# sdmiller/cpu_tsdf

Hardware: AMD Instinct MI355X
Metric: integrateCloud throughput, Scene A turntable depth frames, 640x480 -> voxel grid (higher is better)
Workload: dtype f32

## Files before the change

### cpu_tsdf_amd/csrc/tsdf_common.h

```cpp
#pragma once

#include <hip/hip_runtime.h>
#include <stdint.h>
#include <cmath>
#include <string>
#include <vector>

#include "tsdf_hip.h"

struct tsdf_hip_pipeline;
struct tsdf_hip_multi;
struct tsdf_occ_state;
struct tsdf_meshpost_state;
struct tsdf_flatten_state;
struct tsdf_esdf_state;

struct tsdf_hip_volume {
  tsdf_hip_multi *multi = nullptr;
  tsdf_params p;
  int device = 0;
  int nx = 0, ny = 0, nz = 0;
  int z_begin = 0, z_end = 0;
  int z_first = 0;
  int nz_alloc = 0;
  int64_t pitch = 0;
  int levels[3] = {0, 0, 0};
  float *d = nullptr, *w = nullptr;
  uint32_t *rgb = nullptr;
  uint8_t *k8 = nullptr;
  float *cn[4] = {nullptr, nullptr, nullptr, nullptr};
  float *lab_lut = nullptr;
  float4 *lab_img = nullptr;
  float *vm = nullptr;
  int32_t *vn = nullptr;
  int expf_fused_r = 0;
  float alloc_probe_ms[8] = {-1.f, -1.f, -1.f, -1.f, -1.f, -1.f, -1.f, -1.f};
  int alloc_tried = 0, alloc_chosen = 0;
  int packed = 0;
  unsigned kmax = 0;
  int weight_by_depth = 0, weight_by_variance = 0;
  float *ctr[3] = {nullptr, nullptr, nullptr};
  std::vector<float> h_ctr[3];
  float *frame_depth = nullptr;
  uint32_t *frame_bgra = nullptr;
  uint2 *frame_pairs[2] = {nullptr, nullptr};
  char *bounce = nullptr;
  hipEvent_t bounce_ev[2] = {nullptr, nullptr};
  bool bounce_busy[2] = {false, false};
  unsigned bounce_turn = 0;
  double *cam64 = nullptr;
  tsdf_hip_pipeline *pipe = nullptr;
  int frame_staged = 0;
  uint8_t *band = nullptr;
  int band_fx = 0, band_fy = 0;
  bool band_exact = false;
  int rest_state = 0;
  uint32_t rest_bits = 0;
  unsigned long long last_implied = 0, last_read_bytes = 0;
  bool last_implied_on = false;
  uint8_t *live = nullptr;
  size_t live_cap = 0;
  uint32_t *row_iv = nullptr;
  size_t row_iv_cap = 0;
  bool ctr_increasing[3] = {false, false, false};
  unsigned long long *counter = nullptr;
  unsigned long long last_observed = 0, last_changed_bytes = 0;
  bool ref_cull = false;
  float cull_planes[24] = {0};
// ... 209 lines not shown
int tsdf_shift_band(tsdf_hip_volume *v, int sx, int sy, int sz);
int tsdf_shift_mark(tsdf_hip_volume *v, int which);
void tsdf_shift_clamp(const tsdf_hip_volume *v, const int32_t shift[3], int s[3]);
void tsdf_shift_count(int nx, int ny, int nz, const int s[3], uint64_t *kept, uint64_t *reset);

struct TsdfTuning {
  int rows_per_block;
  int blocks_per_cu;
  int fast_projection;
  int mc_flush_at;
  int mc_skip;
  int cull;
  int vol_chunk;
  int plain_kernel;
  int alloc_tries;
  int allin;
  int refcull_plain;
  int live_log2tx;
  int zfast;
  int fuse2;
  int implied_d;
  int pipe;
  int lab_chunk;
  int frame_pairs;
};
const TsdfTuning &tsdf_tuning();
int tsdf_vol_chunk();

struct PlaneView {
  const float *d, *w;
  const uint32_t *rgb;
  const uint8_t *k8;
  float wmax;
  unsigned kmax;
  int packed;
};

static inline PlaneView tsdf_plane_view(const tsdf_hip_volume *v) {
  return PlaneView{v->d, v->w, v->rgb, v->k8, v->p.max_weight, v->kmax, v->packed};
}

static __device__ __forceinline__ float tsdf_decode_w(unsigned k, float wmax) {
  const float kf = (float)k;
  return kf > wmax ? wmax : kf;
}

// ... 28 lines not shown
```

### cpu_tsdf_amd/csrc/tsdf_core.hip

```cpp
#include <math.h>

#include <string>
#include <stdlib.h>
#include <stdio.h>

#include <algorithm>
#include <thread>
#include <string.h>

#include "tsdf_common.h"
#ifdef TSDF_HIP_TEST_HOOKS
#include "tsdf_hip_test.h"
#endif

static thread_local std::string g_last_error;

void tsdf_set_error(const std::string &msg) { g_last_error = msg; }

int tsdf_hip_fail(hipError_t e, const char *what, const char *file, int line) {
  char buf[512];
  snprintf(buf, sizeof buf, "%s:%d: %s -> %s", file, line, what, hipGetErrorString(e));
  g_last_error = buf;
  (void)hipGetLastError();
  return e == hipErrorOutOfMemory ? TSDF_HIP_E_NOMEM : TSDF_HIP_E_HIP;
}

extern "C" const char *tsdf_hip_last_error(void) { return g_last_error.c_str(); }

extern "C" const char *tsdf_hip_error_string(int code) {
  switch (code) {
    case TSDF_HIP_OK: return "ok";
    case TSDF_HIP_E_INVALID: return "invalid argument";
    case TSDF_HIP_E_NOMEM: return "out of device memory";
    case TSDF_HIP_E_HIP: return "HIP runtime error";
    case TSDF_HIP_E_NODEVICE: return "no HIP device";
    case TSDF_HIP_E_UNSUPPORTED: return "unsupported";
    case TSDF_HIP_E_IO: return "file error";
    case TSDF_HIP_ALIGN_NO_POINTS: return "alignment: no point passed the gate";
    case TSDF_HIP_ALIGN_RANK_DEFICIENT: return "alignment: the cloud does not constrain all six freedoms";
  }
  return "unknown";
}

static int env_int(const char *name, int dflt) {
  const char *e = getenv(name);
  return (e && *e) ? atoi(e) : dflt;
}

static TsdfTuning &tuning_storage() {
  static TsdfTuning t = {std::max(1, env_int("TSDF_HIP_ROWS_PER_BLOCK", 64)),
                         std::max(1, env_int("TSDF_HIP_BLOCKS_PER_CU", 8)),
                         env_int("TSDF_HIP_FAST_PROJECTION", -1), env_int("TSDF_HIP_MC_FLUSH_AT", 512), env_int("TSDF_HIP_MC_SKIP", 1),
                         env_int("TSDF_HIP_CULL", 1), std::max(1, env_int("TSDF_HIP_VOL_CHUNK", 256)),
                         env_int("TSDF_HIP_PLAIN_KERNEL", 0), env_int("TSDF_HIP_ALLOC_TRIES", 3), env_int("TSDF_HIP_ALLIN", 1),
                         env_int("TSDF_HIP_REFCULL_PLAIN", 0), env_int("TSDF_HIP_LIVE_LOG2TX", 5), env_int("TSDF_HIP_ZFAST", 1), env_int("TSDF_HIP_FUSE2", 1), env_int("TSDF_HIP_IMPLIED_D", 1),
                         env_int("TSDF_HIP_PIPE", 1), std::max(1, env_int("TSDF_HIP_LAB_CHUNK", 16 << 20)), env_int("TSDF_HIP_FRAME_PAIRS", 1)};
  return t;
}

const TsdfTuning &tsdf_tuning() { return tuning_storage(); }

int tsdf_vol_chunk() {
  const int live = env_int("TSDF_HIP_VOL_CHUNK", 0);
  return live > 0 ? live : tsdf_tuning().vol_chunk;
}

#ifdef TSDF_HIP_TEST_HOOKS
extern "C" int tsdf_hip_set_tuning(const char *name, int value) {
  if (!name) return TSDF_HIP_E_INVALID;
  TsdfTuning &t = tuning_storage();
  const std::string n(name);
  if (n == "rows_per_block")
    t.rows_per_block = std::max(1, value);
  else if (n == "blocks_per_cu")
    t.blocks_per_cu = std::max(1, value);
  else if (n == "fast_projection")
    t.fast_projection = value;
  else if (n == "mc_flush_at")
    t.mc_flush_at = value;
// ... 5 lines not shown
    t.vol_chunk = std::max(1, value);
  else if (n == "plain_kernel")
    t.plain_kernel = value;
  else if (n == "alloc_tries")
    t.alloc_tries = std::max(1, value);
  else if (n == "allin")
    t.allin = value;
  else if (n == "refcull_plain")
    t.refcull_plain = value;
  else if (n == "fuse2")
    t.fuse2 = value;
  else if (n == "implied_d")
    t.implied_d = value;
  else if (n == "pipe")
    t.pipe = value;
  else if (n == "live_log2tx")
    t.live_log2tx = value;
  else if (n == "zfast")
    t.zfast = value;
  else if (n == "lab_chunk")
    t.lab_chunk = std::max(1, value);
  else if (n == "frame_pairs")
    t.frame_pairs = value;
  else
    return TSDF_HIP_E_INVALID;
  return TSDF_HIP_OK;
}
#endif

extern "C" int tsdf_hip_abi_version(void) { return TSDF_HIP_ABI_VERSION; }

extern "C" int tsdf_hip_host_alloc(size_t bytes, void **out) {
  if (!out || !bytes) return TSDF_HIP_E_INVALID;
  *out = nullptr;
  TSDF_HIP_TRY(hipHostMalloc(out, bytes, hipHostMallocPortable));
  return TSDF_HIP_OK;
}

extern "C" int tsdf_hip_host_free(void *p) {
  if (!p) return TSDF_HIP_OK;
  TSDF_HIP_TRY(hipHostFree(p));
  return TSDF_HIP_OK;
}

extern "C" int tsdf_hip_device_count(void) {
  int n = 0;
// ... 238 lines not shown
  if (!v) return;
  tsdf_occupied_release(v);
  tsdf_meshpost_release(v);
  tsdf_flatten_release(v);
  tsdf_esdf_release(v);
  if (v->multi) tsdf_multi_free(v);
  TsdfDeviceScope scope(v->device);
  tsdf_pipeline_destroy(v);
  if (v->d) (void)hipFree(v->d);
  if (v->w) (void)hipFree(v->w);
  if (v->rgb) (void)hipFree(v->rgb);
  if (v->k8) (void)hipFree(v->k8);
  for (int c = 0; c < 4; ++c)
    if (v->cn[c]) (void)hipFree(v->cn[c]);
  if (v->vm) (void)hipFree(v->vm);
  if (v->vn) (void)hipFree(v->vn);
  if (v->lab_lut) (void)hipFree(v->lab_lut);
  if (v->lab_img) (void)hipFree(v->lab_img);
  for (int a = 0; a < 3; ++a)
    if (v->ctr[a]) (void)hipFree(v->ctr[a]);
  if (v->frame_depth) (void)hipFree(v->frame_depth);
  for (int i = 0; i < 2; ++i)
    if (v->frame_pairs[i]) (void)hipFree(v->frame_pairs[i]);
  if (v->bounce) (void)hipHostFree(v->bounce);
  for (int i = 0; i < 2; ++i)
    if (v->bounce_ev[i]) (void)hipEventDestroy(v->bounce_ev[i]);
  if (v->cam64) (void)hipFree(v->cam64);
  if (v->live) (void)hipFree(v->live);
  if (v->row_iv) (void)hipFree(v->row_iv);
  if (v->band) (void)hipFree(v->band);
  if (v->counter) (void)hipFree(v->counter);
  if (v->mc_verts) (void)hipFree(v->mc_verts);
  if (v->mc_rgb) (void)hipFree(v->mc_rgb);
  if (v->mc_cell) (void)hipFree(v->mc_cell);
  if (v->mc_keys) (void)hipFree(v->mc_keys);
  if (v->mc_vals) (void)hipFree(v->mc_vals);
  if (v->mc_need) (void)hipFree(v->mc_need);
  for (int i = 0; i < 4; ++i)
    if (v->mc_ev[i]) (void)hipEventDestroy(v->mc_ev[i]);
  for (int i = 0; i < 2; ++i)
    if (v->align_ev[i]) (void)hipEventDestroy(v->align_ev[i]);
  for (int i = 0; i < 2; ++i)
    if (v->shift_ev[i]) (void)hipEventDestroy(v->shift_ev[i]);
  for (int i = 0; i < 3; ++i)
    if (v->merge_ev[i]) (void)hipEventDestroy(v->merge_ev[i]);
  if (v->merge_count) (void)hipFree(v->merge_count);
// ... 220 lines not shown
    for (int c = 0; c < (lab ? 3 : 4); ++c) TRY_OR_BAIL(hipMalloc(&v->cn[c], n * sizeof(float)));
  if (lab) {
    float lut[256];
    tsdf_lab_curve(lut);
    TRY_OR_BAIL(hipMalloc(&v->lab_lut, sizeof lut));
    TRY_OR_BAIL(hipMemcpy(v->lab_lut, lut, sizeof lut, hipMemcpyHostToDevice));
    TRY_OR_BAIL(hipMalloc(&v->lab_img, (size_t)p->image_width * p->image_height * sizeof(float4)));
  }
  for (int a = 0; a < 3; ++a) {
    tsdf_build_centers(p->res[a], tsdf_node_size(*p, a), v->h_ctr[a], &v->levels[a]);
    v->ctr_increasing[a] = true;
    for (size_t i = 1; i < v->h_ctr[a].size(); ++i) v->ctr_increasing[a] &= v->h_ctr[a][i - 1] < v->h_ctr[a][i];
    std::vector<float> padded(v->h_ctr[a]);
    padded.resize((size_t)p->res[a] + 4, NAN);
    TRY_OR_BAIL(hipMalloc(&v->ctr[a], padded.size() * sizeof(float)));
    TRY_OR_BAIL(hipMemcpy(v->ctr[a], padded.data(), padded.size() * sizeof(float), hipMemcpyHostToDevice));
  }
  const size_t npx = (size_t)p->image_width * p->image_height;
  TRY_OR_BAIL(hipMalloc(&v->frame_depth, 2 * npx * sizeof(float)));
  v->frame_bgra = reinterpret_cast<uint32_t *>(v->frame_depth + npx);
  if (p->integrate_color)
    for (int i = 0; i < 2; ++i) TRY_OR_BAIL(hipMalloc(&v->frame_pairs[i], 8 * npx));
  {
    const double cam[4] = {p->fx, p->fy, p->cx, p->cy};
    TRY_OR_BAIL(hipMalloc(&v->cam64, sizeof cam));
    TRY_OR_BAIL(hipMemcpy(v->cam64, cam, sizeof cam, hipMemcpyHostToDevice));
  }
  v->band_fx = (v->nx + 63) / 64;
  v->band_fy = (v->ny + 3) / 4;
  TRY_OR_BAIL(hipMalloc(&v->band, (size_t)v->band_fx * v->band_fy * v->nz_alloc));
  TRY_OR_BAIL(hipMalloc(&v->counter, 4096 * sizeof(unsigned long long)));
  TRY_OR_BAIL(hipMemset(v->counter, 0, 4096 * sizeof(unsigned long long)));
#undef TRY_OR_BAIL
  rc = tsdf_hip_reset(v);
  if (rc != TSDF_HIP_OK) return bail(rc);
  *out = v;
  return TSDF_HIP_OK;
}

extern "C" int tsdf_hip_reset(tsdf_handle h) {
  if (!h) return TSDF_HIP_E_INVALID;
  tsdf_normals_invalidate(h);
  if (h->multi) return tsdf_multi_reset(h);
  TSDF_ENTER(h);
  const int64_t n = h->pitch * h->ny * h->nz_alloc;
  const float minus_one = -1.f;
// ... 490 lines not shown
```

### cpu_tsdf_amd/csrc/tsdf_integrate.hip

```cpp
#include <limits.h>
#include <string.h>
#include <math.h>

#include <algorithm>
#include <cmath>
#include <type_traits>

#include "tsdf_common.h"
#include "tsdf_div.h"
#include "tsdf_buffer.h"
#ifdef TSDF_HIP_TEST_HOOKS
#include "tsdf_hip_test.h"
#endif

#ifndef TSDF_WPE_MAX
#define TSDF_WPE_MAX 8
#endif
#ifndef TSDF_WPE_PACKED
#define TSDF_WPE_PACKED 7
#endif
#ifndef TSDF_WPE_PACKED_COLOR
#define TSDF_WPE_PACKED_COLOR 8
#endif
#ifndef TSDF_WPE_GENERAL
#define TSDF_WPE_GENERAL 7
#endif
#ifndef TSDF_WPE_PIPE
#define TSDF_WPE_PIPE 8
#endif
#ifndef TSDF_WPE_PIPEC
#define TSDF_WPE_PIPEC 5
#endif
#ifndef TSDF_WPE_K2
// ... 350 lines not shown
  TSDF_CNT2_READ = 2560,
  TSDF_CNT2_SLOTS = 3072
};
static __device__ __forceinline__ unsigned tsdf_block_number(const BlockCoords &bc) { return bc.bx + bc.by * bc.gdx + bc.bz * bc.gdx * bc.gdy; }
static __device__ __forceinline__ void tsdf_count_out(const BlockCoords &bc, unsigned *s, unsigned long long *n_obs,
                                                      unsigned tid, unsigned cnt, unsigned chg, unsigned imp, unsigned rdb) {
  if (tid == 0) s[0] = s[1] = s[2] = s[3] = 0;
  __syncthreads();
  if (cnt) atomicAdd(&s[0], cnt);
  if (chg) atomicAdd(&s[1], chg);
  if (imp) atomicAdd(&s[2], imp);
  if (rdb) atomicAdd(&s[3], rdb);
  __syncthreads();
  if (tid == 0 && (s[0] || s[3])) {
    const unsigned b = tsdf_block_number(bc) & (TSDF_CNT_STRIPE - 1u);
    if (s[0]) atomicAdd(n_obs + TSDF_CNT_OBSERVED + b, (unsigned long long)s[0]);
    if (s[1]) atomicAdd(n_obs + TSDF_CNT_CHANGED + b, (unsigned long long)s[1]);
    if (s[2]) atomicAdd(n_obs + TSDF_CNT_IMPLIED + b, (unsigned long long)s[2]);
    if (s[3]) atomicAdd(n_obs + TSDF_CNT_READ + b, (unsigned long long)s[3]);
  }
}
#define TSDF_WPE_OF(ORDER, COLOR, FASTPROJ, COUNT, PACKED, ALLIN) \
  ((ALLIN) && !(COUNT) && (PACKED) && (COLOR) && (FASTPROJ) ? TSDF_WPE_PACKED_COLOR : (ALLIN) && !(COUNT) && ((PACKED) || !(COLOR)) ? TSDF_WPE_PACKED : TSDF_WPE_GENERAL)
template <int ORDER, bool COLOR, bool FASTPROJ, bool COUNT, bool PACKED, bool ALLIN = false, bool LIVE = false, bool PAIRS = false>
static __global__ void __launch_bounds__(256) __attribute__((amdgpu_waves_per_eu(TSDF_WPE_OF(ORDER, COLOR, FASTPROJ, COUNT, PACKED, ALLIN) < TSDF_WPE_MAX ? TSDF_WPE_OF(ORDER, COLOR, FASTPROJ, COUNT, PACKED, ALLIN) : TSDF_WPE_MAX, TSDF_WPE_MAX)))
k_integrate(const IntegrateArgs a, float *__restrict__ D, float *__restrict__ Wt, uint32_t *__restrict__ RGB,
            uint8_t *__restrict__ K8, const float *__restrict__ depth, const double *__restrict__ cam,
            const float *__restrict__ ctrx, const float *__restrict__ ctry, const float *__restrict__ ctrz,
            unsigned long long *__restrict__ n_obs, const uint8_t *__restrict__ live, uint8_t *__restrict__ band,
            const uint32_t *__restrict__ row_iv) {
  static_assert(!(ALLIN && LIVE), "the ALLIN instance knows no row intervals");
  static_assert(!PAIRS || COLOR, "pixel records carry the colour: the colourless frame is the depth plane itself");
  const BlockCoords bc = tsdf_block_coords(a.zfast);
  bool strad = false;
  if (LIVE) {
    const unsigned flag = live[bc.bx + bc.gdx * (bc.by + bc.gdy * bc.bz)];
    if (flag == 0u) return;
    strad = flag == 2u;
  }
  const unsigned tid = threadIdx.x;
  __shared__ f2 s_rcp[256];
  __shared__ f4 s_yt[256];
  constexpr bool F2 = ALLIN && FASTPROJ;
  constexpr bool LEAN_K1 = PACKED && COLOR;
  __shared__ f4 s_cx[F2 ? 256 : 1];
  __shared__ uint32_t s_iv[LIVE ? 256 : 1];
  TSDF_BAND_DECL;
  if (PACKED) s_rcp[tid] = tsdf_rcp_entry(a, tid);
  {
    const int yy = (int)bc.by * a.rpb * a.TY + (int)tid;
    const float cy_ = ctry[yy < a.ny ? yy : a.ny - 1], cz_ = ctrz[a.z_global0 + (int)bc.bz];
    f4 t = {0.f, 0.f, 0.f, 0.f};
#pragma unroll
    for (int q = 0; q < 3; ++q) t[q] = tsdf_row_part<ORDER>(a.m, q, cy_, cz_);
    s_yt[tid] = t;
    if (LIVE && strad) s_iv[tid] = yy < a.ny ? row_iv[(int64_t)bc.bz * a.ny + yy] : 0u;
  }
  if (F2) tsdf_park_centres(a, bc, ctrx, s_cx, tid);
  __shared__ uint8_t s_bin[PACKED ? 1024 : 1];
  if (PACKED && a.implied_d) tsdf_flags_before(a, bc, band, s_bin, tid);
  __syncthreads();
  const uint64_t quiet = PACKED && a.implied_d ? tsdf_quiet_passes(a, s_bin, tid) : 0ull;
  const int tx = (int)(tid & (unsigned)(a.TX - 1));
  const int ty = (int)(tid >> a.log2TX);
  const int xq = (int)bc.bx * a.TX + tx;
  const int zl = (int)bc.bz;
  const Rcp32 rneg = rcp32_prepare(a.neg);
  unsigned cnt = 0, chg = 0, imp = 0, rdb = 0;
  const BlockRows br = tsdf_block_rows(a, bc);
  const rsrc_t rsD = make_rsrc(D + br.e0, br.span * 4u);
  const rsrc_t rsW = make_rsrc(PACKED ? D : Wt + br.e0, PACKED ? 0u : br.span * 4u);
  const rsrc_t rsC = make_rsrc(COLOR ? RGB + br.e0 : (uint32_t *)D, COLOR ? br.span * 4u : 0u);
  const rsrc_t rsK = make_rsrc(PACKED && !COLOR ? K8 + br.e0 : (uint8_t *)D, PACKED && !COLOR ? br.span : 0u);
  const unsigned npix = (unsigned)a.W * (unsigned)a.H;
  const rsrc_t rsF = make_rsrc(depth, PAIRS ? npix * 8u : COLOR ? a.bgra_off + npix * 4u : npix * 4u);
  const i4_rsrc rsFi = make_rsrc_2d(depth, PAIRS ? 8u : 4u, 0xffffffffu);
  if (xq < a.qpr) {
    const int x4 = xq * 4;
    const float cz = ctrz[a.z_global0 + zl];
    const float4 cx4 = *reinterpret_cast<const float4 *>(ctrx + x4);
    const float cxs[4] = {cx4.x, cx4.y, cx4.z, cx4.w};
    float px_[4][3], zt[3];
#pragma unroll
    for (int r = 0; r < 3; ++r) {
#pragma unroll
      for (int j = 0; j < 4; ++j) px_[j][r] = cxs[j] * a.m[4 * r];
      zt[r] = ORDER == TSDF_XFORM_PCL_SSE ? cz * a.m[4 * r + 2] + a.m[4 * r + 3] : a.m[4 * r + 2] * cz;
    }
    const unsigned voff = (unsigned)(ty * (int)a.pitch + x4) * 4u;
    const unsigned row_step = (unsigned)a.TY * (unsigned)a.pitch * 4u;
    bool pred_obs = true;
    for (int r = 0; r < a.rpb; ++r) {
      const int y = br.row0 + ty + r * a.TY;
      if (y >= a.ny) break;
      unsigned iv_lo = 0u, iv_len = 0u;
      if (LIVE && strad) {
        const uint32_t iv = s_iv[ty + r * a.TY];
        iv_lo = iv & 0xffffu, iv_len = iv >> 16;
        if (!((unsigned)(x4 + 3) - iv_lo < iv_len + 3u)) continue;
      }
      const unsigned soff = (unsigned)r * row_step;
      const f4 ytv = s_yt[ty + r * a.TY];
      const float yt[3] = {ytv.x, ytv.y, ytv.z};
      float px[4][3];
      if constexpr (!F2) {
        float cxr[4] = {cxs[0], cxs[1], cxs[2], cxs[3]};
#pragma unroll
        for (int j = 0; j < 4; ++j) asm volatile("" : "+v"(cxr[j]));
#pragma unroll
        for (int q = 0; q < 3; ++q)
#pragma unroll
          for (int j = 0; j < 4; ++j) px[j][q] = cxr[j] * a.m[4 * q];
      }
      auto transform = [&](int j, int q) -> float {
        if (ORDER == TSDF_XFORM_PCL_SSE) return px[j][q] + yt[q];
// ... 1553 lines not shown
static __global__ void __launch_bounds__(256)
k_frame_pairs(const uint32_t *__restrict__ depth, const uint32_t *__restrict__ bgra, uint2 *__restrict__ out, unsigned npix) {
  const unsigned i = (blockIdx.x * 256u + threadIdx.x) * 2u;
  if (i + 1u < npix) {
    const uint4 v = {depth[i], bgra[i], depth[i + 1u], bgra[i + 1u]};
    *reinterpret_cast<uint4 *>(out + i) = v;
  } else if (i < npix) {
    out[i] = make_uint2(depth[i], bgra[i]);
  }
}

static int launch_frame_pairs(tsdf_handle h, const float *d_depth, const uint32_t *d_bgra, uint2 *out) {
  const unsigned npix = (unsigned)h->p.image_width * (unsigned)h->p.image_height;
  if (!out || !d_depth || !d_bgra) {
    tsdf_set_error("colour launch without its pixel-record buffer or frame");
    return TSDF_HIP_E_INVALID;
  }
  hipLaunchKernelGGL(k_frame_pairs, dim3((npix + 511u) / 512u), dim3(256), 0, h->stream, reinterpret_cast<const uint32_t *>(d_depth),
                     d_bgra, out, npix);
  TSDF_HIP_TRY(hipGetLastError());
  return TSDF_HIP_OK;
}

static bool frame_pairs_apply(tsdf_handle h) { return tsdf_tuning().frame_pairs && h->p.integrate_color; }

static int zfast_for(const tsdf_params &p, unsigned gx) {
  const size_t frame_bytes = (size_t)p.image_width * p.image_height * (p.integrate_color ? 8 : 4);
  return tsdf_tuning().zfast < 0 ? (frame_bytes > (3u << 20) && gx <= 65535u) : (tsdf_tuning().zfast != 0 && gx <= 65535u);
}

static uint8_t *band_flags_for(tsdf_handle h, const IntegrateArgs &a) {
  uint8_t *band = h->band_exact && ((a.rpb * a.TY) & 3) == 0 && (a.y_abs0 & 3) == 0 ? h->band : nullptr;
  if (!band) h->band_exact = false;
  return band;
}

static bool pipelined_rows_apply(tsdf_handle h, const IntegrateArgs &a, bool color, bool fastproj, bool allin, bool live) {
  return (tsdf_tuning().pipe & (color ? 2 : 1)) && fastproj && allin && !live && h->packed && a.hinge_fixed && a.neg_in_window &&
         a.ny % a.TY == 0;
}

static int launch_plain_family(tsdf_handle h, const IntegrateArgs &a, unsigned gz, int plain_mode, const float *d_depth,
                               const uint32_t *d_bgra, const float T[12], bool count) {
  const tsdf_params &p = h->p;
  if (plain_mode && ((h->packed && plain_mode != 3) || h->cn[0])) {
    tsdf_set_error("weight_by_depth needs the F32W layout and TSDF_COLOR_RGB");
// ... 162 lines not shown
  if (const int e = grow_live_scratch(h, nb, nrows)) return e;
  const dim3 row_grid((unsigned)((nrows + 255) / 256)), block(256);
  if (ra.nx <= TSDF_ROWS_LDS_NX)
    hipLaunchKernelGGL(k_rows<true>, row_grid, block, 0, h->stream, ra, pl.ctrx, pl.ctry, h->ctr[2], h->row_iv);
  else
    hipLaunchKernelGGL(k_rows<false>, row_grid, block, 0, h->stream, ra, pl.ctrx, pl.ctry, h->ctr[2], h->row_iv);
  hipLaunchKernelGGL(k_cull, dim3((unsigned)((nb + 255) / 256)), block, 0, h->stream, c, pl.ctrx, pl.ctry, h->ctr[2], h->row_iv, h->live);
  TSDF_HIP_TRY(hipGetLastError());
  pl.live = h->live;
  return TSDF_HIP_OK;
}

static int plan_live(tsdf_handle h, const float T[12], bool all_inside, bool rc_rows, LaunchPlan &pl) {
  if (!all_inside) narrow_live_blocks(pl);
  if (tsdf_tuning().cull && !all_inside) shrink_to_index_box(h, T, pl);
  if (pl.gy > 65535u) {
    tsdf_set_error("grid too large for one launch");
    return TSDF_HIP_E_UNSUPPORTED;
  }
  return pl.nothing_observable ? TSDF_HIP_OK : launch_rows_and_cull(h, T, rc_rows, pl);
}

static void dispatch_fast(tsdf_handle h, const LaunchPlan &pl, const float *d_depth, bool count, bool fastproj, bool allin,
                          bool pipe, bool pairs, uint8_t *band_arg) {
  const IntegrateArgs &a = pl.a;
  const dim3 grid(a.zfast ? pl.gz : pl.gx, pl.gy, a.zfast ? pl.gx : pl.gz), block(256);
  const bool sse = h->p.xform_order == TSDF_XFORM_PCL_SSE, color = h->p.integrate_color != 0;
  pairs = pairs && color;
  if (pipe) {
    with_consts(
        [&](auto SSE, auto COUNT, auto PAIRS) {
          if (color)
            hipLaunchKernelGGL((k_integrate_pc<xform_order_of(SSE), COUNT, PAIRS>), grid, block, 0, h->stream, a, pl.D, pl.RGB, d_depth,
                               h->cam64, pl.ctrx, pl.ctry, h->ctr[2], h->counter, band_arg);
          else if constexpr (!PAIRS)
            hipLaunchKernelGGL((k_integrate_p<xform_order_of(SSE), COUNT>), grid, block, 0, h->stream, a, pl.D, pl.K8, d_depth,
                               h->cam64, pl.ctrx, pl.ctry, h->ctr[2], h->counter, band_arg);
        },
        sse, count, pairs);
    return;
  }
  with_consts(
      [&](auto SSE, auto COLOR, auto FASTPROJ, auto COUNT, auto PACKED, auto ALLIN, auto LIVE, auto PAIRS) {
        if constexpr (!(ALLIN && (!FASTPROJ || LIVE)) && !(PAIRS && !COLOR))
          hipLaunchKernelGGL((k_integrate<xform_order_of(SSE), COLOR, FASTPROJ, COUNT, PACKED, ALLIN, LIVE, PAIRS>), grid, block, 0,
                             h->stream, a, pl.D, pl.Wt, pl.RGB, pl.K8, d_depth, h->cam64, pl.ctrx, pl.ctry, h->ctr[2], h->counter,
                             pl.live, band_arg, h->row_iv);
      },
      sse, color, fastproj, count, h->packed, allin, pl.live != nullptr, pairs);
}

static int validate_launch(tsdf_handle h, const LaunchPlan &pl, const uint32_t *d_bgra) {
  if (pl.gy > 65535u || pl.gz > 65535u) {
    tsdf_set_error("grid too large for one launch");
    return TSDF_HIP_E_UNSUPPORTED;
  }
  if (h->p.integrate_color && !d_bgra) {
    tsdf_set_error("integrate_color is set but no colour image was given");
    return TSDF_HIP_E_INVALID;
  }
  if (h->weight_by_variance && (!h->vm || !h->vn || h->packed || h->cn[0])) {
    tsdf_set_error("weight_by_variance_ (hpp:203-204) needs the per-voxel M_ / nsample_ planes: F32W layout, TSDF_COLOR_RGB");
    return TSDF_HIP_E_UNSUPPORTED;
  }
  return TSDF_HIP_OK;
}

int tsdf_integrate_launch(tsdf_handle h, const float *d_depth, const uint32_t *d_bgra, const float T[12], bool count) {
  h->count_slots = 0;
  h->count_ran = false;
  const IntegrateHost hh = make_args(h, T);
  LaunchPlan pl = whole_slab_plan(h, hh);
// ... 12 lines not shown
    if (!frame_is_planar(h->p, d_depth, d_bgra)) h->frame_staged = 0;
    a.bgra_off = 0;
  } else if (const int e = stage_frame(h, &d_depth, d_bgra, &a.bgra_off)) {
    return e;
  }
  const LaunchKind kind = launch_kind(h, T, a, rc, rc_rows);
  if (kind.live)
    if (const int e = plan_live(h, T, kind.all_inside, rc_rows, pl)) return e;
  if (count) TSDF_HIP_TRY(hipMemsetAsync(h->counter, 0, TSDF_CNT_SLOTS * sizeof(unsigned long long), h->stream));
  const bool pose_ok = pose_is_finite(T);
  const bool fastproj = fast_projection_ok(hh, h->p.integrate_color != 0);
  h->last_launch[0] = h->last_launch[1] = h->last_launch[2] = h->last_launch[3] = 0;
  uint8_t *band_arg = band_flags_for(h, a);
  a.implied_d = implied_distances(h, a, band_arg != nullptr);
  h->last_implied_on = a.implied_d != 0;
  if (pose_ok && !pl.nothing_observable) {
    const bool live = pl.live != nullptr, allin = fastproj && kind.allin && !live;
    const bool pipe = pipelined_rows_apply(h, a, h->p.integrate_color != 0, fastproj, kind.allin, live);
    a.zfast = zfast_for(h->p, pl.gx);
    h->last_launch[0] = (allin ? 1 : 0) | (pipe ? 0x100 : 0);
    h->last_launch[1] = fastproj;
    h->last_launch[2] = live ? (rc_rows ? 2 : 1) : 0;
    h->last_launch[3] = (int)std::min<uint64_t>((uint64_t)pl.gx * pl.gy * pl.gz, 0x7fffffffu);
    if (pairs) {
      if (const int e = launch_frame_pairs(h, d_depth, d_bgra, h->frame_pairs[0])) return e;
      d_depth = reinterpret_cast<const float *>(h->frame_pairs[0]);
    }
    dispatch_fast(h, pl, d_depth, count, fastproj, allin, pipe, pairs, band_arg);
    TSDF_HIP_TRY(hipGetLastError());
  }
  h->count_slots = count ? TSDF_CNT_SLOTS : 0;
  h->count_ran = pose_ok && !pl.nothing_observable;
  return TSDF_HIP_OK;
}

int tsdf_integrate_collect(tsdf_handle h, uint64_t *n_observed) {
  if (!h->count_slots) {
    tsdf_set_error("tsdf_integrate_collect without a counting launch");
    return TSDF_HIP_E_INVALID;
  }
  unsigned long long c[TSDF_CNT_SLOTS];
  const int slots = h->count_slots;
  TSDF_HIP_TRY(hipMemcpyAsync(c, h->counter, (size_t)slots * sizeof(unsigned long long), hipMemcpyDeviceToHost, h->stream));
  TSDF_HIP_TRY(hipStreamSynchronize(h->stream));
  unsigned long long sum = 0, changed = 0, implied = 0, read_bytes = 0;
  for (int i = TSDF_CNT_OBSERVED; i < TSDF_CNT_CHANGED; ++i) sum += c[i];
  for (int i = TSDF_CNT_CHANGED; i < slots && i < TSDF_CNT_IMPLIED; ++i) changed += c[i];
  for (int i = TSDF_CNT_IMPLIED; i < slots && i < TSDF_CNT_READ; ++i) implied += c[i];
  for (int i = TSDF_CNT_READ; i < slots; ++i) read_bytes += c[i];
  h->last_observed = h->count_ran ? sum : 0;
  h->last_changed_bytes = h->count_ran ? changed : 0;
  h->last_implied = h->count_ran ? implied : 0;
// ... 683 lines not shown
```

Measured before the change: 686,500.

## Skip occluded voxel rows using a max-depth pyramid occlusion test

Builds a hierarchical max-depth pyramid of each depth frame and runs a pre-pass kernel that tests voxel patches against it. For each wave it records the first and last rows that can be visible, and the ALLIN integrate kernel then iterates only over that row range. The aim is to skip voxels lying far behind the observed surface. It adds three extra kernel launches plus a flag readback per frame. An adaptive host heuristic disables the feature for several frames when it stops cutting rows.

```diff
diff --git a/cpu_tsdf_amd/csrc/tsdf_common.h b/cpu_tsdf_amd/csrc/tsdf_common.h
--- a/cpu_tsdf_amd/csrc/tsdf_common.h
+++ b/cpu_tsdf_amd/csrc/tsdf_common.h
@@ -44,6 +44,14 @@
   float *frame_depth = nullptr;
   uint32_t *frame_bgra = nullptr;
   uint2 *frame_pairs[2] = {nullptr, nullptr};
+  uint32_t *hidden_pyr = nullptr;
+  uint32_t *hidden_bounds = nullptr;
+  size_t hidden_bounds_cap = 0;
+  uint32_t *hidden_seen = nullptr, *hidden_flag = nullptr;
+  hipEvent_t hidden_ev = nullptr;
+  uint32_t hidden_id = 0;
+  bool hidden_pending = false;
+  int hidden_idle = 0, hidden_rest = 0;
   char *bounce = nullptr;
   hipEvent_t bounce_ev[2] = {nullptr, nullptr};
   bool bounce_busy[2] = {false, false};
@@ -299,6 +307,7 @@
   int implied_d;
   int pipe;
   int lab_chunk;
+  int hidden_rows;
   int frame_pairs;
 };
 const TsdfTuning &tsdf_tuning();
diff --git a/cpu_tsdf_amd/csrc/tsdf_core.hip b/cpu_tsdf_amd/csrc/tsdf_core.hip
--- a/cpu_tsdf_amd/csrc/tsdf_core.hip
+++ b/cpu_tsdf_amd/csrc/tsdf_core.hip
@@ -9,6 +9,7 @@
 #include <string.h>
 
 #include "tsdf_common.h"
+#include "tsdf_hidden.h"
 #ifdef TSDF_HIP_TEST_HOOKS
 #include "tsdf_hip_test.h"
 #endif
@@ -54,7 +55,7 @@
                          env_int("TSDF_HIP_CULL", 1), std::max(1, env_int("TSDF_HIP_VOL_CHUNK", 256)),
                          env_int("TSDF_HIP_PLAIN_KERNEL", 0), env_int("TSDF_HIP_ALLOC_TRIES", 3), env_int("TSDF_HIP_ALLIN", 1),
                          env_int("TSDF_HIP_REFCULL_PLAIN", 0), env_int("TSDF_HIP_LIVE_LOG2TX", 5), env_int("TSDF_HIP_ZFAST", 1), env_int("TSDF_HIP_FUSE2", 1), env_int("TSDF_HIP_IMPLIED_D", 1),
-                         env_int("TSDF_HIP_PIPE", 1), std::max(1, env_int("TSDF_HIP_LAB_CHUNK", 16 << 20)), env_int("TSDF_HIP_FRAME_PAIRS", 1)};
+                         env_int("TSDF_HIP_PIPE", 1), std::max(1, env_int("TSDF_HIP_LAB_CHUNK", 16 << 20)), env_int("TSDF_HIP_HIDDEN_ROWS", 1), env_int("TSDF_HIP_FRAME_PAIRS", 1)};
   return t;
 }
 
@@ -106,6 +107,8 @@
     t.lab_chunk = std::max(1, value);
   else if (n == "frame_pairs")
     t.frame_pairs = value;
+  else if (n == "hidden_rows")
+    t.hidden_rows = value;
   else
     return TSDF_HIP_E_INVALID;
   return TSDF_HIP_OK;
@@ -390,6 +393,11 @@
   if (v->frame_depth) (void)hipFree(v->frame_depth);
   for (int i = 0; i < 2; ++i)
     if (v->frame_pairs[i]) (void)hipFree(v->frame_pairs[i]);
+  if (v->hidden_pyr) (void)hipFree(v->hidden_pyr);
+  if (v->hidden_bounds) (void)hipFree(v->hidden_bounds);
+  if (v->hidden_seen) (void)hipHostFree(v->hidden_seen);
+  if (v->hidden_flag) (void)hipFree(v->hidden_flag);
+  if (v->hidden_ev) (void)hipEventDestroy(v->hidden_ev);
   if (v->bounce) (void)hipHostFree(v->bounce);
   for (int i = 0; i < 2; ++i)
     if (v->bounce_ev[i]) (void)hipEventDestroy(v->bounce_ev[i]);
@@ -656,6 +664,17 @@
   if (p->integrate_color)
     for (int i = 0; i < 2; ++i) TRY_OR_BAIL(hipMalloc(&v->frame_pairs[i], 8 * npx));
   {
+    uint32_t hdr[TSDF_HIDDEN_HOFF] = {0};
+    const size_t texels = tsdf_hidden_layout(p->image_width, p->image_height, hdr);
+    TRY_OR_BAIL(hipMalloc(&v->hidden_pyr, sizeof hdr + texels * sizeof(float)));
+    TRY_OR_BAIL(hipMemcpy(v->hidden_pyr, hdr, sizeof hdr, hipMemcpyHostToDevice));
+    TRY_OR_BAIL(hipHostMalloc(reinterpret_cast<void **>(&v->hidden_seen), sizeof(uint32_t), hipHostMallocPortable));
+    *v->hidden_seen = 0;
+    TRY_OR_BAIL(hipMalloc(&v->hidden_flag, sizeof(uint32_t)));
+    TRY_OR_BAIL(hipMemset(v->hidden_flag, 0, sizeof(uint32_t)));
+    TRY_OR_BAIL(hipEventCreateWithFlags(&v->hidden_ev, hipEventDisableTiming));
+  }
+  {
     const double cam[4] = {p->fx, p->fy, p->cx, p->cy};
     TRY_OR_BAIL(hipMalloc(&v->cam64, sizeof cam));
     TRY_OR_BAIL(hipMemcpy(v->cam64, cam, sizeof cam, hipMemcpyHostToDevice));
diff --git a/cpu_tsdf_amd/csrc/tsdf_hidden.h b/cpu_tsdf_amd/csrc/tsdf_hidden.h
--- /dev/null
+++ b/cpu_tsdf_amd/csrc/tsdf_hidden.h
@@ -0,0 +1,139 @@
+#pragma once
+#include <math.h>
+#include <stddef.h>
+#include <stdint.h>
+
+#if defined(__HIPCC__)
+#define TSDF_HIDDEN_HD __host__ __device__ __forceinline__
+#else
+#define TSDF_HIDDEN_HD inline
+#endif
+
+enum {
+  TSDF_HIDDEN_HOFF = 32,
+  TSDF_HIDDEN_TILE_LEVELS = 6,
+};
+
+static inline int tsdf_hidden_levels(int W, int H) {
+  int l = TSDF_HIDDEN_TILE_LEVELS;
+  while (l < 24 && (1 << l) < (W > H ? W : H)) ++l;
+  return l;
+}
+static TSDF_HIDDEN_HD int tsdf_hidden_imin(int a, int b) { return a < b ? a : b; }
+static TSDF_HIDDEN_HD int tsdf_hidden_imax(int a, int b) { return a > b ? a : b; }
+static TSDF_HIDDEN_HD int tsdf_hidden_dim(int n, int l) { return (n + (1 << l) - 1) >> l; }
+static inline size_t tsdf_hidden_layout(int W, int H, uint32_t hoff[TSDF_HIDDEN_HOFF]) {
+  const int L = tsdf_hidden_levels(W, H);
+  size_t at = 0;
+  for (int l = 0; l < TSDF_HIDDEN_HOFF; ++l) hoff[l] = 0u;
+  hoff[0] = (uint32_t)L;
+  for (int l = 1; l <= L; ++l) {
+    hoff[l] = (uint32_t)at;
+    at += (size_t)tsdf_hidden_dim(W, l) * (size_t)tsdf_hidden_dim(H, l);
+  }
+  return at;
+}
+static inline void tsdf_hidden_pyramid_host(const float *depth, int W, int H, const uint32_t *hoff, float *tex) {
+  const int L = (int)hoff[0];
+  for (int l = 1; l <= L; ++l) {
+    const int wl = tsdf_hidden_dim(W, l), hl = tsdf_hidden_dim(H, l), wp = l == 1 ? W : tsdf_hidden_dim(W, l - 1),
+              hp = l == 1 ? H : tsdf_hidden_dim(H, l - 1);
+    const float *prev = l == 1 ? depth : tex + hoff[l - 1];
+    for (int y = 0; y < hl; ++y)
+      for (int x = 0; x < wl; ++x) {
+        float m = -INFINITY;
+        for (int dy = 0; dy < 2; ++dy)
+          for (int dx = 0; dx < 2; ++dx) {
+            const int px = 2 * x + dx, py = 2 * y + dy;
+            if (px >= wp || py >= hp) continue;
+            const float v = prev[(size_t)py * wp + px];
+            if (v == v && v > m) m = v;
+          }
+        tex[hoff[l] + (size_t)y * wl + x] = m;
+      }
+  }
+}
+
+struct TsdfHiddenCam {
+  float m[12];
+  float fx, fy, cx, cy;
+  int W, H;
+  float neg, zfloor, zslack;
+  const uint32_t *hoff;
+  const float *tex;
+};
+
+static inline float tsdf_hidden_zslack(const float T[12], const double lo[3], const double hi[3], double fx, double fy) {
+  double big = 0, zmin = 1e300;
+  for (int k = 0; k < 8; ++k) {
+    const double x = (k & 1) ? hi[0] : lo[0], y = (k & 2) ? hi[1] : lo[1], z = (k & 4) ? hi[2] : lo[2];
+    for (int r = 0; r < 3; ++r) {
+      const double g = fabs((double)T[4 * r] * x) + fabs((double)T[4 * r + 1] * y) + fabs((double)T[4 * r + 2] * z) + fabs((double)T[4 * r + 3]);
+      big = g > big ? g : big;
+    }
+    const double gz = (double)T[8] * x + (double)T[9] * y + (double)T[10] * z + (double)T[11];
+    zmin = gz < zmin ? gz : zmin;
+  }
+  const double err = 8.0 * 6e-8 * big, f = fabs(fx) > fabs(fy) ? fabs(fx) : fabs(fy);
+  const bool tight = err < 1e-4 && zmin > 0.05 && f * err * (1.0 + big / zmin) / zmin < 0.05;
+  return tight ? (float)(4.0 * err) : NAN;
+}
+
+static TSDF_HIDDEN_HD void tsdf_hidden_row_part(const TsdfHiddenCam &c, float cy, float cz, float (&ry)[3]) {
+  for (int q = 0; q < 3; ++q) ry[q] = cy * c.m[4 * q + 1] + (cz * c.m[4 * q + 2] + c.m[4 * q + 3]);
+}
+
+struct TsdfHiddenEnd {
+  float u, v, z;
+};
+static TSDF_HIDDEN_HD TsdfHiddenEnd tsdf_hidden_end(const TsdfHiddenCam &c, float x, const float (&ry)[3]) {
+  const float gx = x * c.m[0] + ry[0], gy = x * c.m[4] + ry[1], gz = x * c.m[8] + ry[2];
+#if defined(__HIP_DEVICE_COMPILE__)
+  const float y = __builtin_amdgcn_rcpf(gz);
+#else
+  const float y = 1.f / gz;
+#endif
+  TsdfHiddenEnd e;
+  e.u = gx * c.fx * y + c.cx, e.v = gy * c.fy * y + c.cy, e.z = gz;
+  return e;
+}
+
+template <int N>
+static TSDF_HIDDEN_HD bool tsdf_hidden_hull(const TsdfHiddenCam &c, const TsdfHiddenEnd (&e)[N]) {
+  float zmin = e[0].z, zmax = e[0].z, ulo = e[0].u, uhi = e[0].u, vlo = e[0].v, vhi = e[0].v;
+  bool ok = e[0].z > c.zfloor;
+  float usum = e[0].u, vsum = e[0].v;
+  for (int k = 1; k < N; ++k) {
+    zmin = fminf(zmin, e[k].z), zmax = fmaxf(zmax, e[k].z);
+    ulo = fminf(ulo, e[k].u), uhi = fmaxf(uhi, e[k].u), vlo = fminf(vlo, e[k].v), vhi = fmaxf(vhi, e[k].v);
+    usum += e[k].u, vsum += e[k].v;
+    ok = ok && e[k].z > c.zfloor;
+  }
+  ok = ok && zmax < 1e30f && ulo >= 0.f && vlo >= 0.f && uhi <= (float)(c.W - 1) && vhi <= (float)(c.H - 1) && usum == usum && vsum == vsum;
+  const float fw = (float)(c.W - 1), fh = (float)(c.H - 1);
+  const int x0 = tsdf_hidden_imax((int)fminf(fmaxf(ulo, 0.f), fw) - 1, 0), x1 = tsdf_hidden_imin((int)fminf(fmaxf(uhi, 0.f), fw) + 1, c.W - 1);
+  const int y0 = tsdf_hidden_imax((int)fminf(fmaxf(vlo, 0.f), fh) - 1, 0), y1 = tsdf_hidden_imin((int)fminf(fmaxf(vhi, 0.f), fh) + 1, c.H - 1);
+  const int span = tsdf_hidden_imax(tsdf_hidden_imax(x1 - x0, y1 - y0), 2);
+  const int lw = 32 - __builtin_clz((unsigned)(span - 1)), L = (int)c.hoff[0];
+  ok = ok && lw <= L;
+  const int l = tsdf_hidden_imin(lw, L);
+  const int wl = tsdf_hidden_dim(c.W, l);
+  const float *t = c.tex + c.hoff[l];
+  const int tx0 = x0 >> l, tx1 = x1 >> l, ty0 = (y0 >> l) * wl, ty1 = (y1 >> l) * wl;
+  const float D = fmaxf(fmaxf(t[ty0 + tx0], t[ty0 + tx1]), fmaxf(t[ty1 + tx0], t[ty1 + tx1]));
+  const float B = ((zmin - c.neg) - c.zslack) - 0x1p-20f * (zmin + c.neg);
+  return ok && D < B;
+}
+
+static TSDF_HIDDEN_HD bool tsdf_hidden_segment(const TsdfHiddenCam &c, const float (&p0)[3], const float (&p1)[3]) {
+  float r0[3], r1[3];
+  tsdf_hidden_row_part(c, p0[1], p0[2], r0);
+  tsdf_hidden_row_part(c, p1[1], p1[2], r1);
+  const TsdfHiddenEnd e[2] = {tsdf_hidden_end(c, p0[0], r0), tsdf_hidden_end(c, p1[0], r1)};
+  return tsdf_hidden_hull(c, e);
+}
+
+static TSDF_HIDDEN_HD bool tsdf_hidden_patch(const TsdfHiddenCam &c, float x0, float x1, const float (&ra)[3], const float (&rb)[3]) {
+  const TsdfHiddenEnd e[4] = {tsdf_hidden_end(c, x0, ra), tsdf_hidden_end(c, x1, ra), tsdf_hidden_end(c, x0, rb), tsdf_hidden_end(c, x1, rb)};
+  return tsdf_hidden_hull(c, e);
+}
diff --git a/cpu_tsdf_amd/csrc/tsdf_integrate.hip b/cpu_tsdf_amd/csrc/tsdf_integrate.hip
--- a/cpu_tsdf_amd/csrc/tsdf_integrate.hip
+++ b/cpu_tsdf_amd/csrc/tsdf_integrate.hip
@@ -9,6 +9,7 @@
 #include "tsdf_common.h"
 #include "tsdf_div.h"
 #include "tsdf_buffer.h"
+#include "tsdf_hidden.h"
 #ifdef TSDF_HIP_TEST_HOOKS
 #include "tsdf_hip_test.h"
 #endif
@@ -405,7 +406,7 @@
 }
 #define TSDF_WPE_OF(ORDER, COLOR, FASTPROJ, COUNT, PACKED, ALLIN) \
   ((ALLIN) && !(COUNT) && (PACKED) && (COLOR) && (FASTPROJ) ? TSDF_WPE_PACKED_COLOR : (ALLIN) && !(COUNT) && ((PACKED) || !(COLOR)) ? TSDF_WPE_PACKED : TSDF_WPE_GENERAL)
-template <int ORDER, bool COLOR, bool FASTPROJ, bool COUNT, bool PACKED, bool ALLIN = false, bool LIVE = false, bool PAIRS = false>
+template <int ORDER, bool COLOR, bool FASTPROJ, bool COUNT, bool PACKED, bool ALLIN = false, bool LIVE = false, bool PAIRS = false, bool BOUNDS = false>
 static __global__ void __launch_bounds__(256) __attribute__((amdgpu_waves_per_eu(TSDF_WPE_OF(ORDER, COLOR, FASTPROJ, COUNT, PACKED, ALLIN) < TSDF_WPE_MAX ? TSDF_WPE_OF(ORDER, COLOR, FASTPROJ, COUNT, PACKED, ALLIN) : TSDF_WPE_MAX, TSDF_WPE_MAX)))
 k_integrate(const IntegrateArgs a, float *__restrict__ D, float *__restrict__ Wt, uint32_t *__restrict__ RGB,
             uint8_t *__restrict__ K8, const float *__restrict__ depth, const double *__restrict__ cam,
@@ -414,6 +415,7 @@
             const uint32_t *__restrict__ row_iv) {
   static_assert(!(ALLIN && LIVE), "the ALLIN instance knows no row intervals");
   static_assert(!PAIRS || COLOR, "pixel records carry the colour: the colourless frame is the depth plane itself");
+  static_assert(!BOUNDS || (ALLIN && FASTPROJ), "row bounds travel where the ALLIN instance has no row intervals");
   const BlockCoords bc = tsdf_block_coords(a.zfast);
   bool strad = false;
   if (LIVE) {
@@ -444,6 +446,13 @@
   if (PACKED && a.implied_d) tsdf_flags_before(a, bc, band, s_bin, tid);
   __syncthreads();
   const uint64_t quiet = PACKED && a.implied_d ? tsdf_quiet_passes(a, s_bin, tid) : 0ull;
+  int r_first = 0, r_end = a.rpb;
+  if constexpr (BOUNDS) {
+    if (row_iv) {
+      const uint32_t w = __builtin_amdgcn_readfirstlane(row_iv[(size_t)(bc.bx + bc.gdx * (bc.by + bc.gdy * bc.bz)) * 4u + (tid >> 6)]);
+      r_first = (int)(w & 0xffffu), r_end = (int)(w >> 16);
+    }
+  }
   const int tx = (int)(tid & (unsigned)(a.TX - 1));
   const int ty = (int)(tid >> a.log2TX);
   const int xq = (int)bc.bx * a.TX + tx;
@@ -472,8 +481,8 @@
     }
     const unsigned voff = (unsigned)(ty * (int)a.pitch + x4) * 4u;
     const unsigned row_step = (unsigned)a.TY * (unsigned)a.pitch * 4u;
-    bool pred_obs = true;
-    for (int r = 0; r < a.rpb; ++r) {
+    bool pred_obs = r_first == 0;
+    for (int r = r_first; r < r_end; ++r) {
       const int y = br.row0 + ty + r * a.TY;
       if (y >= a.ny) break;
       unsigned iv_lo = 0u, iv_len = 0u;
@@ -2073,6 +2082,166 @@
   return TSDF_HIP_OK;
 }
 
+static __device__ __forceinline__ float tsdf_depth_or_ninf(uint32_t bits) {
+  const float v = __uint_as_float(bits);
+  return v == v ? v : -INFINITY;
+}
+static __global__ void __launch_bounds__(256)
+k_depth_pyramid(const uint32_t *__restrict__ depth, const uint32_t *__restrict__ hoff, float *__restrict__ tex, int W, int H) {
+  __shared__ float s2[16][16], s3[8][8], s4[4][4], s5[2][2];
+  const int t = (int)threadIdx.x, tx = t & 15, ty = t >> 4;
+  const int px = (int)blockIdx.x * 64 + tx * 4, py = (int)blockIdx.y * 64 + ty * 4;
+  float v[4][4];
+#pragma unroll
+  for (int j = 0; j < 4; ++j)
+#pragma unroll
+    for (int i = 0; i < 4; ++i) v[j][i] = px + i < W && py + j < H ? tsdf_depth_or_ninf(depth[(size_t)(py + j) * (size_t)W + (size_t)(px + i)]) : -INFINITY;
+  const int w1 = tsdf_hidden_dim(W, 1), h1 = tsdf_hidden_dim(H, 1);
+  float m2 = -INFINITY;
+#pragma unroll
+  for (int j = 0; j < 2; ++j)
+#pragma unroll
+    for (int i = 0; i < 2; ++i) {
+      const float m1 = fmaxf(fmaxf(v[2 * j][2 * i], v[2 * j][2 * i + 1]), fmaxf(v[2 * j + 1][2 * i], v[2 * j + 1][2 * i + 1]));
+      const int x1 = (px >> 1) + i, y1 = (py >> 1) + j;
+      if (x1 < w1 && y1 < h1) tex[hoff[1] + (size_t)y1 * w1 + x1] = m1;
+      m2 = fmaxf(m2, m1);
+    }
+  {
+    const int w2 = tsdf_hidden_dim(W, 2), h2 = tsdf_hidden_dim(H, 2), x2 = px >> 2, y2 = py >> 2;
+    if (x2 < w2 && y2 < h2) tex[hoff[2] + (size_t)y2 * w2 + x2] = m2;
+    s2[ty][tx] = m2;
+  }
+  __syncthreads();
+  auto halve = [&](int l, int n, const float *below, float *here) {
+    if (t < n * n) {
+      const int x = t & (n - 1), y = t / n;
+      const float m = fmaxf(fmaxf(below[(2 * y) * 2 * n + 2 * x], below[(2 * y) * 2 * n + 2 * x + 1]),
+                            fmaxf(below[(2 * y + 1) * 2 * n + 2 * x], below[(2 * y + 1) * 2 * n + 2 * x + 1]));
+      const int wl = tsdf_hidden_dim(W, l), hl = tsdf_hidden_dim(H, l), gx = (int)blockIdx.x * n + x, gy = (int)blockIdx.y * n + y;
+      if (gx < wl && gy < hl) tex[hoff[l] + (size_t)gy * wl + gx] = m;
+      if (here) here[y * n + x] = m;
+    }
+  };
+  halve(3, 8, &s2[0][0], &s3[0][0]);
+  __syncthreads();
+  halve(4, 4, &s3[0][0], &s4[0][0]);
+  __syncthreads();
+  halve(5, 2, &s4[0][0], &s5[0][0]);
+  __syncthreads();
+  halve(6, 1, &s5[0][0], nullptr);
+}
+static __global__ void __launch_bounds__(256) k_depth_pyramid_top(const uint32_t *__restrict__ hoff, float *tex, int W, int H) {
+  const int L = (int)hoff[0];
+  for (int l = TSDF_HIDDEN_TILE_LEVELS + 1; l <= L; ++l) {
+    const int wl = tsdf_hidden_dim(W, l), hl = tsdf_hidden_dim(H, l), wp = tsdf_hidden_dim(W, l - 1), hp = tsdf_hidden_dim(H, l - 1);
+    const float *below = tex + hoff[l - 1];
+    for (int i = (int)threadIdx.x; i < wl * hl; i += 256) {
+      const int x = i % wl, y = i / wl;
+      float m = -INFINITY;
+      for (int dy = 0; dy < 2; ++dy)
+        for (int dx = 0; dx < 2; ++dx)
+          if (2 * x + dx < wp && 2 * y + dy < hp) m = fmaxf(m, below[(size_t)(2 * y + dy) * wp + 2 * x + dx]);
+      tex[hoff[l] + i] = m;
+    }
+    __threadfence_block();
+    __syncthreads();
+  }
+}
+
+
+static __global__ void __launch_bounds__(256)
+k_hidden_bounds(const IntegrateArgs a, const TsdfHiddenCam cam, const uint32_t *__restrict__ hdr, const float *__restrict__ ctrx,
+                const float *__restrict__ ctry, const float *__restrict__ ctrz, uint32_t *__restrict__ bounds, uint32_t *seen, uint32_t id) {
+  const unsigned tid = threadIdx.x;
+  const int lane = (int)(tid & 63u), w0 = (int)(tid & ~63u), g = lane >> 2, k = lane & 3;
+  const int n = min(a.rpb, 64);
+  const int pa = min(4 * g, n - 1), pb = min(4 * g + 3, n - 1);
+  const int row0 = (int)blockIdx.y * a.rpb * a.TY + (w0 >> a.log2TX);
+  const int q0 = (int)blockIdx.x * a.TX + (w0 & (a.TX - 1));
+  const int last = a.qpr - 1, qa = q0 + 16 * k;
+  TsdfHiddenCam c = cam;
+  c.hoff = hdr, c.tex = reinterpret_cast<const float *>(hdr + TSDF_HIDDEN_HOFF);
+  const float cz = ctrz[a.z_global0 + (int)blockIdx.z];
+  float ra[3], rb[3];
+  tsdf_hidden_row_part(c, ctry[min(row0 + pa * a.TY, a.ny - 1)], cz, ra);
+  tsdf_hidden_row_part(c, ctry[min(row0 + pb * a.TY, a.ny - 1)], cz, rb);
+  const float x0 = ctrx[4 * min(qa, last)], x1 = ctrx[4 * min(qa + 15, last) + 3];
+  const bool hid = qa > last || tsdf_hidden_patch(c, x0, x1, ra, rb);
+  const uint64_t b = __builtin_amdgcn_ballot_w64(hid);
+  const int ng = (n + 3) >> 2;
+  const uint64_t groups = 0x1111111111111111ull & (ng < 16 ? (1ull << (4 * ng)) - 1ull : ~0ull);
+  const uint64_t vis = ~(b & (b >> 1) & (b >> 2) & (b >> 3)) & groups;
+  const int first = vis ? (int)__builtin_ctzll(vis) : n;
+  const int end = a.rpb > 64 ? a.rpb : vis ? min(a.rpb, 67 - (int)__builtin_clzll(vis)) : 0;
+  if (lane == 0) {
+    bounds[(size_t)(blockIdx.x + gridDim.x * (blockIdx.y + gridDim.y * blockIdx.z)) * 4u + (tid >> 6)] = (uint32_t)first | (uint32_t)end << 16;
+    if ((first > 0 || end < a.rpb) && __hip_atomic_load(seen, __ATOMIC_RELAXED, __HIP_MEMORY_SCOPE_AGENT) != id)
+      __hip_atomic_store(seen, id, __ATOMIC_RELAXED, __HIP_MEMORY_SCOPE_AGENT);
+  }
+}
+
+static int launch_hidden_rows(tsdf_handle h, const float *d_depth, const IntegrateArgs &a, unsigned gx, unsigned gy, unsigned gz,
+                              const float *ctrx, const float *ctry, const TsdfHiddenCam &cam) {
+  const int W = cam.W, H = cam.H;
+  if (!h->hidden_pyr || !d_depth) {
+    tsdf_set_error("hidden-row launch without its pyramid buffer or frame");
+    return TSDF_HIP_E_INVALID;
+  }
+  const size_t words = (size_t)gx * gy * gz * 4;
+  if (words > h->hidden_bounds_cap) {
+    TSDF_HIP_TRY(hipStreamSynchronize(h->stream));
+    if (h->hidden_bounds) TSDF_HIP_TRY(hipFree(h->hidden_bounds));
+    h->hidden_bounds = nullptr, h->hidden_bounds_cap = 0;
+    TSDF_HIP_TRY(hipMalloc(&h->hidden_bounds, words * sizeof(uint32_t)));
+    h->hidden_bounds_cap = words;
+  }
+  float *tex = reinterpret_cast<float *>(h->hidden_pyr + TSDF_HIDDEN_HOFF);
+  hipLaunchKernelGGL(k_depth_pyramid, dim3((unsigned)((W + 63) / 64), (unsigned)((H + 63) / 64)), dim3(256), 0, h->stream,
+                     reinterpret_cast<const uint32_t *>(d_depth), h->hidden_pyr, tex, W, H);
+  if (tsdf_hidden_levels(W, H) > TSDF_HIDDEN_TILE_LEVELS)
+    hipLaunchKernelGGL(k_depth_pyramid_top, dim3(1), dim3(256), 0, h->stream, h->hidden_pyr, tex, W, H);
+  hipLaunchKernelGGL(k_hidden_bounds, dim3(gx, gy, gz), dim3(256), 0, h->stream, a, cam, h->hidden_pyr, ctrx, ctry, h->ctr[2],
+                     h->hidden_bounds, h->hidden_flag, ++h->hidden_id);
+  TSDF_HIP_TRY(hipGetLastError());
+  return TSDF_HIP_OK;
+}
+
+static bool hidden_rows_pay(tsdf_handle h) {
+  if (tsdf_tuning().hidden_rows == 2) return true;
+  if (h->hidden_pending) {
+    const hipError_t q = hipEventQuery(h->hidden_ev);
+    if (q == hipSuccess) {
+      h->hidden_pending = false;
+      const bool cut = *reinterpret_cast<volatile uint32_t *>(h->hidden_seen) == h->hidden_id;
+      h->hidden_idle = cut ? 0 : h->hidden_idle + 1;
+      if (h->hidden_idle >= 4) h->hidden_rest = 7;
+    } else {
+      (void)hipGetLastError();
+    }
+  }
+  if (h->hidden_rest > 0) {
+    --h->hidden_rest;
+    return false;
+  }
+  return true;
+}
+
+static bool hidden_rows_apply(tsdf_handle h, const float T[12], const IntegrateArgs &a, TsdfHiddenCam *cam) {
+  if (!tsdf_tuning().hidden_rows || !h->hidden_pyr || !h->hidden_seen || !h->hidden_flag || !h->hidden_ev || a.log2TX < 6 || !h->ctr_increasing[0] ||
+      !h->ctr_increasing[1] || !h->ctr_increasing[2])
+    return false;
+  if (!hidden_rows_pay(h)) return false;
+  const double lo[3] = {h->h_ctr[0][0], h->h_ctr[1][0], h->h_ctr[2][h->z_begin]},
+               hi[3] = {h->h_ctr[0][h->nx - 1], h->h_ctr[1][h->ny - 1], h->h_ctr[2][h->z_end - 1]};
+  TsdfHiddenCam &c = *cam;
+  for (int i = 0; i < 12; ++i) c.m[i] = a.m[i];
+  c.fx = a.fxf, c.fy = a.fyf, c.cx = a.cxf, c.cy = a.cyf, c.W = a.W, c.H = a.H;
+  c.neg = a.neg, c.zfloor = 1e-3f, c.zslack = tsdf_hidden_zslack(T, lo, hi, h->p.fx, h->p.fy);
+  c.hoff = nullptr, c.tex = nullptr;
+  return c.zslack == c.zslack;
+}
+
 static bool frame_pairs_apply(tsdf_handle h) { return tsdf_tuning().frame_pairs && h->p.integrate_color; }
 
 static int zfast_for(const tsdf_params &p, unsigned gx) {
@@ -2281,7 +2450,7 @@
 }
 
 static void dispatch_fast(tsdf_handle h, const LaunchPlan &pl, const float *d_depth, bool count, bool fastproj, bool allin,
-                          bool pipe, bool pairs, uint8_t *band_arg) {
+                          bool pipe, bool pairs, uint8_t *band_arg, bool hidden) {
   const IntegrateArgs &a = pl.a;
   const dim3 grid(a.zfast ? pl.gz : pl.gx, pl.gy, a.zfast ? pl.gx : pl.gz), block(256);
   const bool sse = h->p.xform_order == TSDF_XFORM_PCL_SSE, color = h->p.integrate_color != 0;
@@ -2299,14 +2468,15 @@
         sse, count, pairs);
     return;
   }
+  const uint32_t *rows_arg = allin ? (hidden ? h->hidden_bounds : nullptr) : h->row_iv;
   with_consts(
-      [&](auto SSE, auto COLOR, auto FASTPROJ, auto COUNT, auto PACKED, auto ALLIN, auto LIVE, auto PAIRS) {
-        if constexpr (!(ALLIN && (!FASTPROJ || LIVE)) && !(PAIRS && !COLOR))
-          hipLaunchKernelGGL((k_integrate<xform_order_of(SSE), COLOR, FASTPROJ, COUNT, PACKED, ALLIN, LIVE, PAIRS>), grid, block, 0,
+      [&](auto SSE, auto COLOR, auto FASTPROJ, auto COUNT, auto PACKED, auto ALLIN, auto LIVE, auto PAIRS, auto BOUNDS) {
+        if constexpr (!(ALLIN && (!FASTPROJ || LIVE)) && !(PAIRS && !COLOR) && !(BOUNDS && !ALLIN))
+          hipLaunchKernelGGL((k_integrate<xform_order_of(SSE), COLOR, FASTPROJ, COUNT, PACKED, ALLIN, LIVE, PAIRS, BOUNDS>), grid, block, 0,
                              h->stream, a, pl.D, pl.Wt, pl.RGB, pl.K8, d_depth, h->cam64, pl.ctrx, pl.ctry, h->ctr[2], h->counter,
-                             pl.live, band_arg, h->row_iv);
+                             pl.live, band_arg, rows_arg);
       },
-      sse, color, fastproj, count, h->packed, allin, pl.live != nullptr, pairs);
+      sse, color, fastproj, count, h->packed, allin, pl.live != nullptr, pairs, allin && hidden);
 }
 
 static int validate_launch(tsdf_handle h, const LaunchPlan &pl, const uint32_t *d_bgra) {
@@ -2365,12 +2535,24 @@
     h->last_launch[1] = fastproj;
     h->last_launch[2] = live ? (rc_rows ? 2 : 1) : 0;
     h->last_launch[3] = (int)std::min<uint64_t>((uint64_t)pl.gx * pl.gy * pl.gz, 0x7fffffffu);
+    TsdfHiddenCam hid_cam;
+    bool hidden = false;
+    if (allin && !pipe && hidden_rows_apply(h, T, a, &hid_cam)) {
+      if (const int e = launch_hidden_rows(h, d_depth, a, pl.gx, pl.gy, pl.gz, pl.ctrx, pl.ctry, hid_cam)) return e;
+      hidden = true;
+      h->last_launch[0] |= 0x200;
+    }
     if (pairs) {
       if (const int e = launch_frame_pairs(h, d_depth, d_bgra, h->frame_pairs[0])) return e;
       d_depth = reinterpret_cast<const float *>(h->frame_pairs[0]);
     }
-    dispatch_fast(h, pl, d_depth, count, fastproj, allin, pipe, pairs, band_arg);
+    dispatch_fast(h, pl, d_depth, count, fastproj, allin, pipe, pairs, band_arg, hidden);
     TSDF_HIP_TRY(hipGetLastError());
+    if (hidden) {
+      TSDF_HIP_TRY(hipMemcpyAsync(h->hidden_seen, h->hidden_flag, sizeof(uint32_t), hipMemcpyDeviceToHost, h->stream));
+      TSDF_HIP_TRY(hipEventRecord(h->hidden_ev, h->stream));
+      h->hidden_pending = true;
+    }
   }
   h->count_slots = count ? TSDF_CNT_SLOTS : 0;
   h->count_ran = pose_ok && !pl.nothing_observable;
```

Result: faster. 697,500, median of 6 (+1.6%).
